# Pablete1234/parquet-floor

Measured on AMD Instinct MI355X. Metric: decoded GB/s + rows/s (node), lineitem-shape Snappy+dict, 1/2/4/8 GPUs, higher is better.
Workload: dtype u8; 1 GPU; lineitem SF1 x1 (6001215 rows x 1, 16 cols, 6 row groups of 1Mi rows), Snappy + dictionary, device-resident; row_groups_per_rank=6, compressed_page_bytes_rank0=217870360

## Files before the change

### parquet-floor_amd/csrc/pf_internal.h

```cpp
#pragma once
#include <stdint.h>

namespace pf {

struct PfOpts {
    int exec = 5;
    bool ba_fused = true;
    bool page_null = false;
    bool null_dict_lds = true;
    int null_stagger = 0;
    bool nest_timeout = false;
    uint32_t null_dcap = 0;
    bool piece_order = true;
    unsigned debug_skip = 0;
    int force_serial = 0;
    int force_redo = 0;
    bool exec_stream = false;
    bool zc = true;
    bool dl_kernel = true;
    bool h2d_kernel = false;
    int h2d_grid = 256;
    bool dl_stream = true;
    bool dl_prio = false;
    bool debug_plan = false;
    int64_t nest_seg = 0;
    bool nest_seg_set = false;
    bool dbp_par = true;
    int fix_shift = 1;
    int decode_grid = 32;
    int count_grid = 64;
};

enum : int32_t {
    PG_V2 = 1,
    PG_COMPRESSED = 2,
    PG_DICT = 4,
};

struct SnappyJob {
    const uint8_t* src;
// ... 116 lines not shown

constexpr uint32_t RT_CAP = 1024;
constexpr uint32_t RT_BYTES = 16 + 8 * RT_CAP;

constexpr uint32_t LT_BLOCK_RUNS = 512;
constexpr uint32_t LT_BT_WORDS = 8;
constexpr uint32_t NL_DST = 4096;
constexpr uint32_t NULL_DICT_LDS = 16384;
constexpr uint32_t NL_IST = 12288;
constexpr uint32_t NL_SLACK = 256;
struct NullCaps {
    uint32_t dcap, icap, dlds;
};
__host__ __device__ inline uint32_t lvl_table_cap(int32_t num_values) {
    return uint32_t(num_values) / 8u + 64u;
}

enum : int32_t { BA_OK = 0, BA_FALLBACK = 1, BA_SKIP = 2, BA_RELINK = 3 };
struct BaJob {
    const uint8_t* p;
    uint32_t* pos;
    uint32_t* len;
    int64_t* chars_out;
    uint32_t* cand;
    uint32_t* link1;
    uint32_t* link2;
    uint32_t* tile_cnt;
    int64_t count;
    uint32_t n;
    uint32_t n_cap;
    uint32_t n_tiles;
    int32_t chunk, page;
    int32_t state;
};

struct DevChunk {
    int32_t ptype, type_length, width, max_def, max_rep, repeated_def, list_null_def, codec;
    int32_t dict_page;
    int32_t first_page;
    int32_t n_pages;
    int32_t needs_count;
    int64_t num_entries;
    const uint8_t* dict_data;
    uint32_t* dict_pos;
    uint32_t* dict_len;
    int64_t dict_n;
    uint8_t* values;
    uint8_t* validity;
    int32_t* offsets;
    uint8_t* chars;
    int32_t* list_offsets;
    uint8_t* list_validity;
    uint8_t* def_levels;
    uint8_t* rep_levels;
    int64_t values_cap, chars_cap, slots_cap, rows_cap;
};

struct DevChunkResult {
    int64_t num_slots, num_values, num_rows, num_chars;
    int32_t status;
    int32_t err_page;
};

struct ScanChunk {
    const uint8_t* base;
    uint64_t size;
    int64_t num_values;
// ... 21 lines not shown
```

### parquet-floor_amd/csrc/pf_pages.hip

```cpp
#include <hip/hip_runtime.h>

#include "pf_device.h"
#include "pf_snappy_par.h"

namespace pf {

constexpr int NT = 256;

#ifdef PF_STAMPS
__device__ unsigned long long pf_pstamps[16];
#define PSTAMP(i, v) atomicAdd(&pf_pstamps[i], (unsigned long long)(v))
extern "C" int pf_debug_pstamps(unsigned long long* out, int n, int reset) {
    if (hipMemcpyFromSymbol(out, HIP_SYMBOL(pf_pstamps), sizeof(unsigned long long) * (n < 16 ? n : 16)) != hipSuccess) return -1;
    if (reset) {
        unsigned long long z[16] = {};
        if (hipMemcpyToSymbol(HIP_SYMBOL(pf_pstamps), z, sizeof z) != hipSuccess) return -1;
    }
    return 0;
}
#else
#define PSTAMP(i, v) ((void)0)
#endif
#ifndef PF_TILE
#define PF_TILE 512
// ... 529 lines not shown
            const uint32_t r = uint32_t(x - sb), ww = r >> 5;
            const uint32_t word = (C[ww] & L2[ww]) >> (r & 31u);
            const int64_t span = min(int64_t(32 - (r & 31u)), stop - x);
            if (word & (span >= 32 ? 0xffffffffu : ((1u << span) - 1u))) { bad = true; break; }
            x += span;
        }
        if (!bad && sv < wend && sv < int64_t(n)) {
            const uint32_t r = uint32_t(sv - sb);
            bad = !(((C[r >> 5] & L2[r >> 5]) >> (r & 31u)) & 1u);
        }
    }
    uint32_t tot;
    block_excl_scan<NT>(__popc(acc), tmp, tot);
    if (threadIdx.x == 0) J.tile_cnt[jt.y] = tot;
    if (__syncthreads_or(bad) && threadIdx.x == 0) atomicExch(&J.state, int32_t(BA_RELINK));
}

__global__ __launch_bounds__(NT) void k_ba_count(BaJob* __restrict__ jobs, const int2* __restrict__ tiles) {
    __shared__ uint32_t tmp[NT / 64];
    const int2 jt = tiles[blockIdx.x];
    const BaJob& J = jobs[jt.x];
    if (J.state != BA_OK) return;
    const uint32_t t0 = uint32_t(jt.y) * BA_TILE;
    if (t0 >= J.n) {
        if (threadIdx.x == 0) J.tile_cnt[jt.y] = 0;
        return;
    }
    const uint32_t wi = t0 / 32 + threadIdx.x;
    uint32_t tot;
    block_excl_scan<NT>(__popc(J.cand[wi] & J.link2[wi]), tmp, tot);
    if (threadIdx.x == 0) J.tile_cnt[jt.y] = tot;
}

__global__ __launch_bounds__(NT) void k_ba_scan(BaJob* __restrict__ jobs, int32_t fail_state) {
    __shared__ uint32_t tmp[NT / 64];
    BaJob& J = jobs[blockIdx.x];
    if (J.state != BA_OK) return;
    uint64_t run = 0;
    for (uint32_t b = 0; b < J.n_tiles; b += NT) {
        const uint32_t i = b + threadIdx.x;
        const uint32_t v = i < J.n_tiles ? J.tile_cnt[i] : 0u;
        uint32_t tot;
        const uint32_t ex = block_excl_scan<NT>(v, tmp, tot);
        if (i < J.n_tiles) J.tile_cnt[i] = uint32_t(run) + ex;
        run += tot;
    }
    if (threadIdx.x == 0 && int64_t(run) != J.count) {
        J.state = fail_state;
        PSTAMP(14, 1);
        PSTAMP(15, run > uint64_t(J.count) ? run - uint64_t(J.count) : 0);
    }
}

__global__ __launch_bounds__(NT) void k_ba_emit(BaJob* __restrict__ jobs, const int2* __restrict__ tiles) {
    __shared__ uint32_t tmp[NT / 64];
    const int2 jt = tiles[blockIdx.x];
    const BaJob& J = jobs[jt.x];
    if (J.state != BA_OK) return;
    const uint32_t n = J.n;
    const uint32_t t0 = uint32_t(jt.y) * BA_TILE;
    if (t0 >= n) return;
    const uint32_t wi = t0 / 32 + threadIdx.x;
    uint32_t m = J.cand[wi] & J.link2[wi];
    uint32_t tot;
    uint64_t k = uint64_t(J.tile_cnt[jt.y]) + block_excl_scan<NT>(__popc(m), tmp, tot);
    const uint64_t count = uint64_t(J.count);
    while (m) {
        const uint32_t q = wi * 32u + uint32_t(__ffs(m) - 1);
        m &= m - 1;
        if (k < count) {
            J.pos[k] = q + 4;
            if (J.len || k + 1 == count) {
                const uint32_t l = ld32le(J.p, q, n);
                if (J.len) J.len[k] = l;
                if (k + 1 == count && J.chars_out) *J.chars_out = int64_t(q) + 4 + int64_t(l) - 4 * int64_t(count);
            }
        }
        k++;
    }
}

__global__ __launch_bounds__(NT) void k_ba_verify(BaJob* __restrict__ jobs, const int2* __restrict__ tiles) {
    __shared__ uint32_t tmp[NT / 64];
    const int2 jt = tiles[blockIdx.x];
    BaJob& J = jobs[jt.x];
    if (J.state != BA_OK) return;
    const uint32_t n = J.n;
    const uint32_t t0 = uint32_t(jt.y) * BA_TILE;
    if (t0 >= n) return;
    const uint32_t wi = t0 / 32 + threadIdx.x;
    uint32_t m = J.cand[wi] & J.link2[wi];
// ... 93 lines not shown
    return 0;
}
#define BA_COUNT(i) (threadIdx.x == 0 ? (void)atomicAdd(&pf_ba_counts[i], 1ull) : (void)0)
#else
#define BA_COUNT(i) ((void)0)
#endif
__global__ __launch_bounds__(NT) void k_ba_fallback(BaJob* __restrict__ jobs, int n_jobs, DevChunkResult* res) {
    __shared__ BinWalkLds W;
    __shared__ long long s_chars;
    for (int j = blockIdx.x; j < n_jobs; j += gridDim.x) {
        BaJob& J = jobs[j];
        if (J.state == BA_RELINK) {
            if (threadIdx.x == 0) s_chars = 0;
            __syncthreads();
            const int64_t c = ba_relink_wg(J, W.scan);
            if (c > 0) atomicAdd(reinterpret_cast<unsigned long long*>(&s_chars), (unsigned long long)c);
            __syncthreads();
            if (c >= 0) {
                if (threadIdx.x == 0 && J.chars_out) *J.chars_out = s_chars;
                BA_COUNT(0);
                __syncthreads();
                continue;
            }
        } else if (J.state != BA_FALLBACK) {
            continue;
        }
        const int64_t t = binary_walk_wg(J.p, J.n, J.count, J.pos, J.len, W);
        BA_COUNT(1);
        if (threadIdx.x == 0) {
            if (t < 0) set_status(res, J.chunk, ST_CORRUPT, J.page);
            else if (J.chars_out) *J.chars_out = t;
        }
        __syncthreads();
    }
}

constexpr uint32_t DSTR_CAP = 256;
constexpr uint32_t FBLK = 4096;

__device__ __forceinline__ uint64_t* flat_block_chars(const DevPage& pg) {
    if (!pg.aux) return nullptr;
    const uintptr_t a = reinterpret_cast<uintptr_t>(pg.aux + pg.aux_cap + 1);
    return reinterpret_cast<uint64_t*>((a + 7) & ~uintptr_t(7));
}
__device__ __forceinline__ bool is_dict_enc(int e) { return e == 2 || e == 8; }

struct CountLds {
    LevelLds L;
    Piece pval[TILE];
    uint32_t ids[TILE];
    uint32_t scan_tmp[NT / 64];
    RleState sval;
    int npval, verr;
    unsigned long long chars_acc;
};

__device__ void count_page(const DevChunk* __restrict__ chunks, DevPage* pages, int pi, DevChunkResult* res, BaJob* bajobs,
                           CountLds& C) {
    LevelLds& L = C.L;
    Piece* pval = C.pval;
    uint32_t* ids = C.ids;
    uint32_t* scan_tmp = C.scan_tmp;
    RleState& sval = C.sval;
    int& npval = C.npval;
    int& verr = C.verr;
    unsigned long long& chars_acc = C.chars_acc;
// ... 1507 lines not shown
        }
        __syncthreads();
    }
    const bool direct = dval & (jf <= FB_WHOLE);
    const int err = flat_present_fixed(S, ck, pg, s, dict, boolean, enc, w, ids, ids_n, id_bw,
                                       uint64_t(pg.entry_start), e_begin, e_end, direct);
#ifdef PF_STAMPS
    if (tid == 0) { const unsigned long long dt_ = __builtin_amdgcn_s_memtime() - ft0; PSTAMP(1, dt_); PSTAMP(0, 1); atomicMax(&pf_pstamps[9], dt_); }
#endif
    if (tid == 0) {
        if (err) set_status(res, pg.chunk, ST_CORRUPT, pi);
        else if (ck.needs_count == 0)
            atomicAdd(reinterpret_cast<unsigned long long*>(&res[pg.chunk].num_values), (unsigned long long)(e_end - e_begin));
        atomicOr(&pg.done, DONE_FIXED);
    }
    return true;
}

__device__ __forceinline__ void null_fallback(int* fbq, int2 pbk) {
    if (threadIdx.x == 0) reinterpret_cast<int2*>(fbq + 4)[atomicAdd(fbq, 1)] = pbk;
}

#ifndef PF_FIXED_OCC
#define PF_FIXED_OCC 6
#endif
__global__ __launch_bounds__(NT, PF_FIXED_OCC) void k_flat_fixed(const DevChunk* __restrict__ chunks, DevPage* pages,
                                                              const int2* __restrict__ blocks, DevChunkResult* res, int* fbq) {
    __shared__ FixedLds S;
    const int2 pbk = blocks[blockIdx.x];
    if (!flat_fixed_block(S, chunks, pages, pbk, res)) null_fallback(fbq, pbk);
}

__device__ __forceinline__ void flat_block(FlatLds& S, const DevChunk* __restrict__ chunks, DevPage* pages, const int2 pbk,
                           DevChunkResult* res) {
    if (pbk.x < 0) return;
    const int pi = pbk.x;
    const uint32_t blk = uint32_t(pbk.y) & 0x0fffffffu;
    const uint32_t bsz = FBLK << (uint32_t(pbk.y) >> 28);
    DevPage& pg = pages[pi];
    const DevChunk& ck = chunks[pg.chunk];
    const int tid = threadIdx.x;
    if ((res[pg.chunk].status != 0) | (ck.max_rep != 0) | ((pg.done & (DONE_FIXED | DONE_NULL)) != 0)) return;
    Sections s;
    if (!page_sections(pg, ck, s)) return;
    const int enc = pg.encoding;
    const bool binary = ck.ptype == 6, boolean = ck.ptype == 0, dict = is_dict_enc(enc);
    const int w = ck.width;
    bool take = ck.max_def == 0 || s.def_rle;
    if (enc == 0) {
    } else if (dict) take = take && !boolean;
    else if (enc == 5) take = take && (ck.ptype == 1 || ck.ptype == 2) && pg.aux != nullptr;
    else take = false;
    if (!take) return;

    const int bwd = bit_width(ck.max_def);
    const uint32_t ne = uint32_t(pg.num_values);
    const int id_bw = (dict && s.val_n > 0) ? int(s.val[0]) : 0;
    const uint8_t* ids = dict && s.val_n > 0 ? s.val + 1 : s.val;
    const uint64_t ids_n = dict && s.val_n > 0 ? s.val_n - 1 : 0;
    const bool counted = ck.needs_count != 0;
    const uint64_t slot_base = uint64_t(pg.entry_start);
    if (blk > 0 && blk * bsz >= ne) return;
    const uint32_t* T = pg.runtab;
    uint32_t t0 = 0, t3 = 0;
    if (T != nullptr) { t0 = T[0]; t3 = T[3]; }
    const bool tab = (t3 == 1u) & (t0 <= uint32_t(RUN_CAP));
    if (tid == 0) S.allp = tab ? 1 : (ck.max_def == 0 ? 1 : all_present(s.def, s.def_n, bwd, ne, uint32_t(ck.max_def)));
    __syncthreads();
    const bool split = S.allp;
    if (!split && blk > 0) return;
    const uint32_t e_begin = split ? blk * bsz : 0u;
    const uint32_t e_end = split ? min(ne, e_begin + bsz) : ne;
#ifdef PF_STAMPS
    const unsigned long long ft0 = __builtin_amdgcn_s_memtime();
    if (tid == 0) { PSTAMP(0, 1); if (dict) PSTAMP(6, 1); if (binary) PSTAMP(7, 1); }
// ... 240 lines not shown
            else copy_chars_fast(S.coff, S.csrc, tv, tchars, sb, se, ck.chars + char_base, S.cv);
        }
        FSTAMP(15);
        if (ck.max_def > 0 && ck.validity) flush_bits(S.vbits, slot_base + e0, want, ck.validity);
        vidx += tv;
        char_base += tchars;
        __syncthreads();
#ifdef PF_STAMPS
        { const unsigned long long t_ = __builtin_amdgcn_s_memtime(); if (tid == 0) PSTAMP(5, t_ - ft1); ft1 = t_; }
#endif
    }
#ifdef PF_STAMPS
    if (tid == 0) {
        const unsigned long long dt_ = __builtin_amdgcn_s_memtime() - ft0;
        PSTAMP(1, dt_);
        atomicMax(&pf_pstamps[binary ? 8 : 9], dt_);
        if (!split) PSTAMP(10, 1);
    }
#endif
    if (tid == 0) {
        if (err) set_status(res, pg.chunk, ST_CORRUPT, pi);
        else if (!counted) atomicAdd(reinterpret_cast<unsigned long long*>(&res[pg.chunk].num_values),
                                     (unsigned long long)(vidx - e_begin));
        atomicOr(&pg.done, DONE_FLAT);
    }
}


#ifndef PF_FLAT_OCC
#define PF_FLAT_OCC 5
#endif
__global__ __launch_bounds__(NT, PF_FLAT_OCC) void k_flat_all(const DevChunk* __restrict__ chunks, DevPage* pages,
                                                 const int2* __restrict__ blocks, int n, const int* __restrict__ fbq,
                                                 DevChunkResult* res) {
    __shared__ union FlatAllLds {
        FixedLds f;
        FlatLds g;
    } S;
    if (int(blockIdx.x) >= n) {
        const int nq = fbq[0], g = int(gridDim.x) - n;
        for (int i = int(blockIdx.x) - n; i < nq; i += g) {
            const int2 pq = reinterpret_cast<const int2*>(fbq + 4)[i];
            if (!flat_fixed_block(S.f, chunks, pages, pq, res)) {
                __syncthreads();
                flat_block(S.g, chunks, pages, pq, res);
            }
            __syncthreads();
        }
        return;
    }
    const int2 pbk = blocks[blockIdx.x];
    if (flat_fixed_block(S.f, chunks, pages, pbk, res)) return;
    __syncthreads();
    flat_block(S.g, chunks, pages, pbk, res);
}

constexpr uint32_t LVL_STAGE = 4096;

__device__ __forceinline__ uint32_t lds_bits(const uint8_t* st, uint32_t bit, uint32_t k) {
    const uint32_t* w = reinterpret_cast<const uint32_t*>(st);
    const uint32_t wi = bit >> 5, sh = bit & 31u;
    const uint64_t v = uint64_t(w[wi]) | (uint64_t(w[wi + 1]) << 32);
    return uint32_t(v >> sh) & (k >= 32 ? 0xffffffffu : ((1u << k) - 1u));
}

__device__ __forceinline__ uint32_t lvl_run_at(const uint32_t* runs, uint32_t nr, uint32_t e) {
    uint32_t lo = 0, hi = nr;
    while (hi - lo > 1) {
        const uint32_t m = (lo + hi) >> 1;
        if (runs[4 * m] <= e) lo = m; else hi = m;
    }
    return lo;
}
__device__ inline uint32_t lvl_values_before(const uint32_t* runs, uint32_t r, uint32_t e, const uint8_t* stage,
                                             uint32_t woff, int bw, uint32_t maxd) {
    const uint32_t first = runs[4 * r], data = runs[4 * r + 1], cw = runs[4 * r + 2];
    const uint32_t before = e - first;
    uint32_t vb = runs[4 * r + 3];
    if (!(cw >> 31)) return vb + (data == maxd ? before : 0u);
    if (bw == 1) {
        for (uint32_t i = 0; i < before; i += 32) {
            const uint32_t k = min(32u, before - i), bb = woff * 8u + data + i;
            if (bb + k <= LVL_STAGE * 8u) vb += __popc(lds_bits(stage, bb, k));
        }
    } else {
        for (uint32_t i = 0; i < before; i++) {
            const uint32_t bb = woff * 8u + data + i * uint32_t(bw);
// ... 1305 lines not shown
    hipLaunchKernelGGL(k_count_seg, dim3(n_segs), dim3(NT), 0, st, d_chunks, d_pages, d_segs, d_res);
    hipLaunchKernelGGL(k_nest_scan, dim3(n), dim3(64), 0, st, d_chunks, d_pages, d_list, d_res);
    hipLaunchKernelGGL(k_nest_ids, dim3(n_segs), dim3(NT), 0, st, d_chunks, d_pages, d_segs, d_res);
    hipLaunchKernelGGL(k_nest_chars, dim3(n), dim3(64), 0, st, d_chunks, d_pages, d_list, d_res);
}
void launch_nest_decode(const DevChunk* d_chunks, DevPage* d_pages, const int2* d_segs, int n_segs, DevChunkResult* d_res,
                        hipStream_t st) {
    if (n_segs > 0) hipLaunchKernelGGL(k_decode_seg, dim3(n_segs), dim3(NT), 0, st, d_chunks, d_pages, d_segs, d_res);
}
void launch_count(const DevChunk* d_chunks, DevPage* d_pages, const int* d_list, int n, int n_flat, const int2* d_dblk, int n_dblk,
                  DevChunkResult* d_res, BaJob* d_bajobs, hipStream_t st, int idle_grid) {
    if (n <= 0) return;
    if (n_dblk > 0) hipLaunchKernelGGL(k_count_dict, dim3(n_dblk), dim3(NT), 0, st, d_chunks, d_pages, d_dblk, d_res);
    if (n_flat > 0) hipLaunchKernelGGL(k_count_flat, dim3(n_flat), dim3(NT), 0, st, d_chunks, d_pages, d_list, d_res, d_bajobs);
    hipLaunchKernelGGL(k_count, dim3(std::min(n, idle_grid)), dim3(NT), 0, st, d_chunks, d_pages, d_list, n, d_res, d_bajobs);
}
void launch_ba(BaJob* d_jobs, int n_jobs, const int2* d_tiles, int n_tiles, DevChunkResult* d_res, hipStream_t st,
               bool short_values) {
    if (n_jobs <= 0 || n_tiles <= 0) return;
    const bool fused = short_values;
    if (!fused) {
        hipLaunchKernelGGL(k_ba_cand, dim3(n_tiles), dim3(NT), 0, st, d_jobs, d_tiles);
        hipLaunchKernelGGL(k_ba_link, dim3(n_tiles), dim3(NT), 0, st, d_jobs, d_tiles, 1);
        hipLaunchKernelGGL(k_ba_link, dim3(n_tiles), dim3(NT), 0, st, d_jobs, d_tiles, 2);
        hipLaunchKernelGGL(k_ba_count, dim3(n_tiles), dim3(NT), 0, st, d_jobs, d_tiles);
    } else {
        hipLaunchKernelGGL(k_ba_tile, dim3(n_tiles), dim3(NT), 0, st, d_jobs, d_tiles);
    }
    hipLaunchKernelGGL(k_ba_scan, dim3(n_jobs), dim3(NT), 0, st, d_jobs, fused ? int32_t(BA_RELINK) : int32_t(BA_FALLBACK));
    hipLaunchKernelGGL(k_ba_emit, dim3(n_tiles), dim3(NT), 0, st, d_jobs, d_tiles);
    if (!fused) hipLaunchKernelGGL(k_ba_verify, dim3(n_tiles), dim3(NT), 0, st, d_jobs, d_tiles);
    hipLaunchKernelGGL(k_ba_fallback, dim3(std::min(n_jobs, 64)), dim3(NT), 0, st, d_jobs, n_jobs, d_res);
}
#ifdef PF_DIAG
__global__ __launch_bounds__(64) void k_debug_walk(const uint8_t* p, uint64_t n, int bw, uint32_t lo, uint32_t limit, int cap,
                                                    uint32_t pos0, uint32_t first0, uint32_t* out) {
    __shared__ Run R[RUN_CAP];
    __shared__ int s_nr;
    __shared__ uint32_t s_cov;
    __shared__ RunWalk s_st;
    const int tid = threadIdx.x;
    uint32_t* o1 = out;
    uint32_t* o2 = out + 5 + 4 * cap;
    if (tid == 0) {
        RunWalk st{pos0, first0};
        int nr = 0;
        uint32_t cov = 0;
        const int r = walk_runs(p, n, bw, lo, limit, R, cap, nr, cov, st);
        o1[0] = uint32_t(r); o1[1] = uint32_t(nr); o1[2] = cov; o1[3] = uint32_t(st.pos); o1[4] = st.first;
        for (int i = 0; i < nr; i++) { o1[5 + 4 * i] = R[i].first; o1[6 + 4 * i] = R[i].count; o1[7 + 4 * i] = R[i].data; o1[8 + 4 * i] = R[i].packed; }
        s_st = RunWalk{pos0, first0};
    }
    __syncthreads();
    const int r = wave_walk_runs(p, n, bw, lo, limit, R, cap, s_nr, s_cov, s_st, RunWalk{pos0, first0});
    __syncthreads();
    if (tid == 0) {
        o2[0] = uint32_t(r); o2[1] = uint32_t(s_nr); o2[2] = s_cov; o2[3] = uint32_t(s_st.pos); o2[4] = s_st.first;
    }
    for (int i = tid; i < s_nr; i += 64) { o2[5 + 4 * i] = R[i].first; o2[6 + 4 * i] = R[i].count; o2[7 + 4 * i] = R[i].data; o2[8 + 4 * i] = R[i].packed; }
}

extern "C" int pf_debug_walk_runs(const uint8_t* stream, uint64_t n, int bw, uint32_t lo, uint32_t limit, int cap,
                                  uint32_t pos0, uint32_t first0, uint32_t* out) {
    if (cap > int(RUN_CAP) || cap < 0) return -1;
    uint8_t* d = nullptr;
    uint32_t* o = nullptr;
// ... 53 lines not shown
                d[b] = g[tab[2 * k] + (b - tab[2 * k + 1])];
            }
        }
    }
}
void launch_snappy_litcopy(const SnappyJob* d_jobs, const int* d_list, int n, const int* d_fb, hipStream_t st) {
    if (n > 0) hipLaunchKernelGGL(k_snappy_litcopy, dim3(n, LC_SPLIT), dim3(NT), 0, st, d_jobs, d_list, d_fb);
}
void launch_snappy_head(SnappyJob* d_jobs, int n_jobs, DevPage* d_pages, const DevChunk* d_chunks, int* d_fb,
                        const DevChunkResult* d_res, hipStream_t st) {
    if (n_jobs > 0)
        hipLaunchKernelGGL(k_snappy_head, dim3((n_jobs + 63) / 64), dim3(64), 0, st, d_jobs, n_jobs, d_pages, d_chunks, d_fb,
                           d_res);
}
void launch_scan(DevChunk* d_chunks, DevPage* d_pages, const int* d_list, int n, DevChunkResult* d_res,
                 uint8_t* arena, uint64_t cap, unsigned long long* used, hipStream_t st) {
    if (n > 0) hipLaunchKernelGGL(k_scan, dim3(n), dim3(64), 0, st, d_chunks, d_pages, d_list, d_res, arena, cap, used);
}
void launch_runs(const DevChunk* d_chunks, DevPage* d_pages, const int* d_list, int n, DevChunkResult* d_res,
                 hipStream_t st) {
    if (n > 0) hipLaunchKernelGGL(k_runs, dim3(n), dim3(128), 0, st, d_chunks, d_pages, d_list, d_res);
}
void launch_lvl(const DevChunk* d_chunks, DevPage* d_pages, const int* d_list, int n, DevChunkResult* d_res,
                hipStream_t st, bool page_null, NullCaps nc) {
    if (n <= 0) return;
#ifdef PF_DIAG
    if (page_null) hipLaunchKernelGGL(k_page_null, dim3(n), dim3(PN_NT), 0, st, d_chunks, d_pages, d_list, d_res);
#else
    (void)page_null;
#endif
    hipLaunchKernelGGL(k_lvl, dim3(n), dim3(LT_NT), 0, st, d_chunks, d_pages, d_list, d_res, nc.dcap, nc.icap);
}
void launch_flat(const DevChunk* d_chunks, DevPage* d_pages, const int* d_list, int nfix, int n, int n4, int n8, int* d_fbq,
                 DevChunkResult* d_res, hipStream_t st, NullCaps nc, int stagger) {
    const int2* blocks = reinterpret_cast<const int2*>(d_list);
    const size_t dyn = size_t(nc.dcap) + 32u + nc.icap + 32u + nc.dlds;
    if (n4 > 0)
        hipLaunchKernelGGL(k_flat_null<4>, dim3(n4), dim3(NTN), dyn, st, d_chunks, d_pages, blocks + nfix + n, d_res, nc, stagger, d_fbq);
    if (n8 > 0)
        hipLaunchKernelGGL(k_flat_null<8>, dim3(n8), dim3(NTN), dyn, st, d_chunks, d_pages, blocks + nfix + n + n4, d_res, nc, stagger,
                           d_fbq);
    if (nfix > 0) hipLaunchKernelGGL(k_flat_fixed, dim3(nfix), dim3(NT), 0, st, d_chunks, d_pages, blocks, d_res, d_fbq);
    const int nq = nfix + n4 + n8;
    const int nqw = nq < 32 ? nq : 32;
    if (n + nqw > 0)
        hipLaunchKernelGGL(k_flat_all, dim3(n + nqw), dim3(NT), 0, st, d_chunks, d_pages, blocks + nfix, n, d_fbq, d_res);
}
void launch_decode(const DevChunk* d_chunks, DevPage* d_pages, const int* d_list, int n, int n_first,
                   DevChunkResult* d_res, hipStream_t st, int idle_grid) {
    const int g = std::min(n, std::max(idle_grid, n_first));
    if (n > 0) hipLaunchKernelGGL(k_decode, dim3(g), dim3(NT), 0, st, d_chunks, d_pages, d_list, n, d_res);
}

}
```

### parquet-floor_amd/csrc/pf_runtime.hip

```cpp
#include <hip/hip_runtime.h>

#include <algorithm>
#include <chrono>
#include <cstdio>
#include <cstdlib>
#include <cstring>
#include <memory>
#include <mutex>
#include <string>
#include <vector>

#include "pf_encode.h"
#include "pf_host.h"
#include "pf_snappy_par.h"
#include "pfloor.h"

namespace pf {
void launch_snappy(const SnappyJob*, int, const int2*, int, SnapWin*, SnapEnt*, uint32_t*, const int2*, int, uint32_t*,
                   int*, DevChunkResult*, int, int, hipStream_t);
void launch_snappy_parse(const SnappyJob*, int, const int2*, int, SnapWin*, SnapEnt*, uint32_t*, uint32_t*, int*, int,
                         hipStream_t);
void launch_snappy_exec(const SnappyJob*, int, const int2*, int, uint32_t*, int*, DevChunkResult*, int, hipStream_t);
void launch_ba(BaJob*, int, const int2*, int, DevChunkResult*, hipStream_t, bool);
void launch_snappy_head(SnappyJob*, int, DevPage*, const DevChunk*, int*, const DevChunkResult*, hipStream_t);
void launch_snappy_litcopy(const SnappyJob*, const int*, int, const int*, hipStream_t);
void launch_delta(const DevChunk*, DevPage*, const int*, int, int, DevChunkResult*, hipStream_t);
void launch_dlen(const DevChunk*, DevPage*, const int*, int, DevChunkResult*, hipStream_t);
void launch_dba_chars(const DevChunk*, DevPage*, const int*, int, DevChunkResult*, hipStream_t);
void launch_count(const DevChunk*, DevPage*, const int*, int, int, const int2*, int, DevChunkResult*, BaJob*, hipStream_t, int);
void launch_scan(DevChunk*, DevPage*, const int*, int, DevChunkResult*, uint8_t*, uint64_t, unsigned long long*, hipStream_t);
void launch_flat(const DevChunk*, DevPage*, const int*, int, int, int, int, int*, DevChunkResult*, hipStream_t, NullCaps, int);
void launch_lvl(const DevChunk*, DevPage*, const int*, int, DevChunkResult*, hipStream_t, bool, NullCaps);
void launch_runs(const DevChunk*, DevPage*, const int*, int, DevChunkResult*, hipStream_t);
void launch_decode(const DevChunk*, DevPage*, const int*, int, int, DevChunkResult*, hipStream_t, int);
void launch_nest_lvl(const DevChunk*, DevPage*, const int*, int, int, DevChunkResult*, hipStream_t, bool);
void launch_nest_count(const DevChunk*, DevPage*, const int*, int, const int2*, int, DevChunkResult*, hipStream_t);
void launch_nest_decode(const DevChunk*, DevPage*, const int2*, int, DevChunkResult*, hipStream_t);
void launch_page_scan(const ScanChunk*, int, pf_page_desc*, ScanCrc*, ScanResult*, hipStream_t);
void launch_page_crc(const ScanCrc*, const int*, int, ScanResult*, int32_t*, hipStream_t);
}

using namespace pf;

namespace {

thread_local std::string g_err;

int fail(pf_ctx* ctx, int code, const std::string& msg);

struct DevBuf {
    void* p = nullptr;
    size_t cap = 0;
    hipError_t ensure(size_t n) {
        if (n <= cap) return hipSuccess;
        if (p) { (void)hipFree(p); p = nullptr; cap = 0; }
        size_t want = std::max<size_t>(n + n / 4, 1 << 20);
        hipError_t e = hipMalloc(&p, want);
        if (e == hipSuccess) cap = want;
        return e;
    }
    void release() { if (p) (void)hipFree(p); p = nullptr; cap = 0; }
};

struct HostBuf {
// ... 90 lines not shown
    int device = 0;
    pf::PfOpts opts;
    std::shared_ptr<Streams> streams;
    hipStream_t stream = nullptr;
    hipStream_t exec_stream = nullptr;
    hipEvent_t ev_fork = nullptr, ev_join = nullptr;
    bool zc = true;
    hipEvent_t ev[N_EVENTS] = {};
    hipEvent_t ev_done = nullptr;
    hipEvent_t ev_copy = nullptr;
    hipEvent_t ev_dl = nullptr;
    bool timing = true;
    std::string err;
    DevBuf d_in, d_scratch, d_out, d_bits, d_chars, d_meta, d_tokmap;
    DevBuf d_scan_in, d_scan;
    DevBuf d_enc, d_enc_sec, d_enc_out;
    std::vector<uint8_t> h_enc;
    HostBuf h_meta, h_res;
    HostBuf h_enc_slots;
    int n_chunks = 0;
    bool pending = false;
    bool copies_pending = false;
    bool tables_from_decode = false;
    bool timing_valid = false;
    std::vector<DevChunk> chunks;
    std::vector<DevPage> pages;
    std::vector<SnappyJob> jobs;
    std::vector<int> l_dictbin, l_delta, l_count, l_scan, l_flat, l_decode, l_runs, l_dlen, l_dba, l_lvl, l_djobs, l_nest, l_nseg,
        l_cdict;
    std::vector<int2> wins, pieces;
    std::vector<BaJob> bajobs;
    std::vector<int2> ba_tiles;
    int n_ba_dict = 0, n_ba_dict_tiles = 0;
    bool ba_short_dict = true, ba_short_data = true;
    uint32_t null_dict_lds = 0;
    bool meta_by_kernel = false;
    uint32_t null_dcap = 16, null_icap = 16;
    int max_snap_win = 1;
    uint32_t n_splits = 0;
    SnapWin* d_win = nullptr;
    SnapEnt* d_ent = nullptr;
    const uint32_t* d_last_splits = nullptr;
    uint32_t* d_lane_out = nullptr;
    std::vector<int64_t> host_status;
    std::vector<pf_column_info> info;
    size_t bits_bytes = 0;
    int n_decode_first = 0;
    int n_count_flat = 0;
    int n_flat_fixed = 0, n_flat_all = 0, n_null4 = 0, n_null8 = 0;
    size_t off_npub = 0, npub_bytes = 0;
    int max_nwin = 0, max_dbp_nwin = 0;
    size_t out_bytes = 0;
    size_t off_chunks = 0, off_pages = 0, off_jobs = 0, off_lists = 0, off_res = 0, meta_bytes = 0;
    size_t off_pieces = 0, off_splits = 0, off_fallback = 0, off_wins = 0, off_bajobs = 0, off_batiles = 0, off_nfbq = 0;
    uint64_t chars_need = 0;
    const uint8_t* d_bytes = nullptr;
    int reruns = 0;
};

namespace {

int fail(pf_ctx* ctx, int code, const std::string& msg) {
    if (ctx) ctx->err = msg;
    g_err = msg;
    return code;
}
// ... 76 lines not shown
                           ctx->opts.exec, ctx->exec_stream);
        HIPCHK(ctx, hipEventRecord(ctx->ev_join, ctx->exec_stream));
        HIPCHK(ctx, hipStreamWaitEvent(st, ctx->ev_join, 0));
    } else {
        launch_snappy_exec(d_jobs, int(ctx->jobs.size()), d_pieces, int(ctx->pieces.size()), d_splits, d_fallback, d_res,
                           ctx->opts.exec, st);
    }
    EVREC(ctx, ctx->ev[3], st);
    BaJob* d_bajobs = reinterpret_cast<BaJob*>(meta + ctx->off_bajobs);
    const int2* d_batiles = reinterpret_cast<const int2*>(meta + ctx->off_batiles);
    const int n_ba = int(ctx->bajobs.size()), n_bt = int(ctx->ba_tiles.size());
    (void)d_dictbin;
    if (!(skip & 4u)) launch_ba(d_bajobs, ctx->n_ba_dict, d_batiles, ctx->n_ba_dict_tiles, d_res, st, ctx->ba_short_dict && ctx->opts.ba_fused);
    EVREC(ctx, ctx->ev[4], st);
    launch_delta(d_chunks, d_pages, d_delta, int(ctx->l_delta.size()), ctx->max_dbp_nwin, d_res, st);
    EVREC(ctx, ctx->ev[5], st);
    if (!(skip & 8u)) launch_runs(d_chunks, d_pages, d_runs, int(ctx->l_runs.size()), d_res, st);
    const NullCaps ncaps{ctx->opts.null_dcap ? ctx->opts.null_dcap : ctx->null_dcap, ctx->null_icap,
                         ctx->opts.null_dict_lds ? ctx->null_dict_lds : 0u};
    if (!(skip & 8u)) launch_lvl(d_chunks, d_pages, d_lvl, int(ctx->l_lvl.size()), d_res, st, ctx->opts.page_null, ncaps);
    launch_dlen(d_chunks, d_pages, d_dlen, int(ctx->l_dlen.size()), d_res, st);
    EVREC(ctx, ctx->ev[6], st);
    launch_nest_lvl(d_chunks, d_pages, d_nest, n_nest, ctx->max_nwin, d_res, st, ctx->opts.nest_timeout);
    if (!(skip & 16u)) launch_count(d_chunks, d_pages, d_count, int(ctx->l_count.size()), ctx->n_count_flat, d_cdict, int(ctx->l_cdict.size() / 2),
                                       d_res, d_bajobs, st, ctx->opts.count_grid);
    launch_nest_count(d_chunks, d_pages, d_nest, n_nest, d_nseg, n_nseg, d_res, st);
    if (!(skip & 4u))
        launch_ba(d_bajobs + ctx->n_ba_dict, n_ba - ctx->n_ba_dict, d_batiles + ctx->n_ba_dict_tiles, n_bt - ctx->n_ba_dict_tiles,
                  d_res, st, ctx->ba_short_data && ctx->opts.ba_fused);
    EVREC(ctx, ctx->ev[7], st);
    launch_scan(d_chunks, d_pages, d_scan, int(ctx->l_scan.size()), d_res, static_cast<uint8_t*>(ctx->d_chars.p),
                ctx->d_chars.cap, used, st);
    EVREC(ctx, ctx->ev[8], st);
    if (!(skip & 32u))
        launch_flat(d_chunks, d_pages, d_flat, ctx->n_flat_fixed, ctx->n_flat_all, ctx->n_null4, ctx->n_null8,
                    reinterpret_cast<int*>(meta + ctx->off_nfbq), d_res, st, ncaps, ctx->opts.null_stagger);
    EVREC(ctx, ctx->ev[9], st);
    if (!(skip & 64u)) launch_decode(d_chunks, d_pages, d_decode, int(ctx->l_decode.size()), ctx->n_decode_first, d_res, st,
                                       ctx->opts.decode_grid);
    launch_nest_decode(d_chunks, d_pages, d_nseg, n_nseg, d_res, st);
    launch_dba_chars(d_chunks, d_pages, d_dba, int(ctx->l_dba.size()), d_res, st);
    EVREC(ctx, ctx->ev[10], st);
    HIPCHK(ctx, hipGetLastError());
    const size_t res_pad = align_up(sizeof(DevChunkResult) * ctx->n_chunks, 256);
    if (ctx->zc && ctx->h_res.d) {
        copy_words(ctx->h_res.d, meta + ctx->off_res, sizeof(DevChunkResult) * ctx->n_chunks,
                   static_cast<uint8_t*>(ctx->h_res.d) + res_pad, d_chunks, sizeof(DevChunk) * ctx->n_chunks, st);
    } else {
        HIPCHK(ctx, hipMemcpyAsync(ctx->h_res.p, meta + ctx->off_res, sizeof(DevChunkResult) * ctx->n_chunks,
                                   hipMemcpyDeviceToHost, st));
        HIPCHK(ctx, hipMemcpyAsync(static_cast<uint8_t*>(ctx->h_res.p) + res_pad, d_chunks, sizeof(DevChunk) * ctx->n_chunks,
                                   hipMemcpyDeviceToHost, st));
    }
    HIPCHK(ctx, hipEventRecord(ctx->ev_done, st));
    return PF_OK;
}

int plan_snappy(pf_ctx* ctx) {
    ctx->wins.clear();
    ctx->pieces.clear();
    ctx->n_splits = 0;
    ctx->max_snap_win = 1;
    uint32_t n_win = 0;
    size_t tw = 0, tp = 0;
    for (SnappyJob& jb : ctx->jobs) {
        jb.n_win = std::max<uint32_t>(1u, uint32_t((uint64_t(jb.src_len) + SNAP_WIN - 1) / SNAP_WIN));
        ctx->max_snap_win = std::max(ctx->max_snap_win, int(std::min<uint32_t>(jb.n_win, 1u << 20)));
        jb.n_pieces = std::max<uint32_t>(1u, uint32_t((uint64_t(jb.dst_len) + SNAP_BLOCK - 1) / SNAP_BLOCK));
        tw += jb.n_win;
// ... 424 lines not shown
    out->encode_ms = enc_ms;
    out->snappy_in = 0;
    out->snappy_out = 0;
    if (col->codec == PF_CODEC_SNAPPY)
        for (size_t i = 0; i < sections.size(); i++) {
            out->snappy_in += int64_t(sections[i].second);
            out->snappy_out += int64_t(bodies[i].size());
        }
    return PF_OK;
}

extern "C" {

int pf_abi_version(void) { return PF_ABI_VERSION; }

const char* pf_last_error(pf_ctx* ctx) { return ctx ? ctx->err.c_str() : g_err.c_str(); }

int pf_device_count(int* count) {
    if (!count) return fail(nullptr, PF_ERR_INVALID_ARG, "null count");
    int n = 0;
    hipError_t e = hipGetDeviceCount(&n);
    if (e != hipSuccess) { *count = 0; return fail(nullptr, PF_ERR_HIP, hipGetErrorString(e)); }
    *count = n;
    return PF_OK;
}

namespace {
#ifdef PF_DIAG
void opts_from_env(pf::PfOpts& o) {
    auto on = [](const char* name, bool dflt) { const char* e = std::getenv(name); return e ? e[0] == '1' : dflt; };
    auto num = [](const char* name, int dflt) { const char* e = std::getenv(name); return e ? std::atoi(e) : dflt; };
    o.exec = num("PF_EXEC", o.exec);
    o.ba_fused = on("PF_BA_FUSED", o.ba_fused);
    o.page_null = on("PF_PAGE_NULL", o.page_null);
    o.null_dict_lds = on("PF_NULL_DICT_LDS", o.null_dict_lds);
    o.nest_timeout = on("PF_DEBUG_NEST_TIMEOUT", o.nest_timeout);
    o.null_dcap = uint32_t(std::max(0, num("PF_NULL_DCAP", 0))) & ~15u;
    o.null_stagger = num("PF_DEBUG_NULL_STAGGER", o.null_stagger);
    o.piece_order = on("PF_PIECE_ORDER", o.piece_order);
    if (const char* e = std::getenv("PF_DEBUG_SKIP")) {
        const char* names[] = {"parse", "exec", "ba", "levels", "count", "flat", "decode"};
        for (int i = 0; i < 7; i++)
            if (std::strstr(e, names[i])) o.debug_skip |= 1u << i;
    }
    o.force_serial = num("PF_DEBUG_FORCE_SERIAL", o.force_serial);
    o.force_redo = num("PF_DEBUG_FORCE_REDO", o.force_redo);
    o.exec_stream = on("PF_EXEC_STREAM", o.exec_stream);
    o.zc = on("PF_ZC", o.zc);
    o.dl_kernel = on("PF_DL_KERNEL", o.dl_kernel);
    o.dl_stream = on("PF_DL_STREAM", o.dl_stream);
    o.h2d_kernel = on("PF_H2D_KERNEL", o.h2d_kernel);
    o.h2d_grid = std::max(1, num("PF_H2D_GRID", o.h2d_grid));
    o.dl_prio = on("PF_DL_PRIO", o.dl_prio);
    o.debug_plan = on("PF_DEBUG_PLAN", o.debug_plan);
    if (const char* e = std::getenv("PF_NEST_SEG")) {
        o.nest_seg = std::atoll(e);
        o.nest_seg_set = true;
    }
    o.dbp_par = on("PF_DBP_PAR", o.dbp_par);
    o.decode_grid = std::max(1, num("PF_DECODE_GRID", o.decode_grid));
    o.count_grid = std::max(1, num("PF_COUNT_GRID", o.count_grid));
    const int fb = num("PF_FIX_BLK", 8192);
    o.fix_shift = fb >= 16384 ? 2 : (fb >= 8192 ? 1 : 0);
}
#endif

// ... 299 lines not shown
                            }
                        }
                    }
                }
                pplan.push_back(pp);
                ctx->pages.push_back(pg);
            }
        }
        if (hs != 0) {
            while (int(ctx->pages.size()) > ck.first_page) { ctx->pages.pop_back(); pplan.pop_back(); }
            while (!ctx->jobs.empty() && ctx->jobs.back().chunk == c) ctx->jobs.pop_back();
            if (!ctx->l_dictbin.empty() && ctx->l_dictbin.back() == c) ctx->l_dictbin.pop_back();
            ck.n_pages = 0; ck.dict_page = -1; entries = 0;
        }
        if (ck.dict_page >= 0) ck.first_page = ck.dict_page + 1;
        ck.num_entries = entries;
        OutPlan& op = oplan[c];
        op = OutPlan{~size_t(0), ~size_t(0), ~size_t(0), ~size_t(0), ~size_t(0), ~size_t(0), ~size_t(0)};
        if (hs == 0) {
            if (ck.width > 0) op.values = take(out, size_t(entries) * ck.width);
            if (cd.max_def > 0) op.validity = take(bits, align_up((entries + 7) / 8, 4), 256);
            if (cd.physical_type == PF_BYTE_ARRAY) op.offsets = take(out, 4 * size_t(entries + 1));
            if (cd.max_rep == 1) {
                op.list_offsets = take(out, 4 * size_t(entries + 1));
                op.list_validity = take(bits, align_up((entries + 7) / 8, 4), 256);
            }
            if (cd.max_rep > 0) { op.def = take(out, entries); op.rep = take(out, entries); }
        }
    }
    mark();
    ctx->bajobs.clear();
    ctx->ba_tiles.clear();
    ctx->ba_short_dict = ctx->ba_short_data = true;
    constexpr uint64_t BA_SHORT = 48;
    std::vector<size_t> ba_bm;
    for (int pass = 0; pass < 2; pass++) {
        for (size_t i = 0; i < ctx->pages.size(); i++) {
            DevPage& pg = ctx->pages[i];
            const DevChunk& ck = ctx->chunks[pg.chunk];
            if (ck.ptype != PF_BYTE_ARRAY || ctx->host_status[pg.chunk] != 0) continue;
            const bool is_dict = pg.flags & PG_DICT;
            if (pass == 0 ? !is_dict : (is_dict || pg.encoding != PF_ENC_PLAIN)) continue;
            BaJob J{};
            J.n_cap = pg.body_len;
            J.n_tiles = std::max<uint32_t>(1u, (pg.body_len + BA_TILE_BYTES - 1) / BA_TILE_BYTES);
            J.chunk = pg.chunk;
            J.page = int32_t(i);
            J.state = BA_SKIP;
            const size_t words = size_t(J.n_tiles) * (BA_TILE_BYTES / 32);
            ba_bm.push_back(take(scratch, 4 * (3 * words + J.n_tiles), 256));
            const int rel = int(ctx->bajobs.size()) - (pass == 0 ? 0 : ctx->n_ba_dict);
            for (uint32_t t = 0; t < J.n_tiles; t++) ctx->ba_tiles.push_back(int2{rel, int(t)});
            if (pass == 1) pg.ba_job = int32_t(ctx->bajobs.size());
            if (uint64_t(pg.body_len) > BA_SHORT * uint64_t(std::max<int64_t>(1, pg.num_values)))
                (pass == 0 ? ctx->ba_short_dict : ctx->ba_short_data) = false;
            ctx->bajobs.push_back(J);
        }
        if (pass == 0) { ctx->n_ba_dict = int(ctx->bajobs.size()); ctx->n_ba_dict_tiles = int(ctx->ba_tiles.size()); }
    }
    mark();
    size_t chars_cap = std::max<size_t>(size_t(2 * chars_hint) + (16u << 20), ctx->chars_need);
    if (ctx->copies_pending) {
        if (out > ctx->d_out.cap || bits > ctx->d_bits.cap || chars_cap > ctx->d_chars.cap)
            HIPCHK(ctx, hipEventSynchronize(ctx->ev_copy));
        else
            HIPCHK(ctx, hipStreamWaitEvent(st, ctx->ev_copy, 0));
// ... 66 lines not shown
            if (pp.dx_off != ~0ull) {
                pg.dx = reinterpret_cast<uint64_t*>(S + pp.dx_off);
                ctx->l_dlen.push_back(int(i));
                if (pg.encoding == PF_ENC_DELTA_BYTE_ARRAY) ctx->l_dba.push_back(int(i));
            }
            DevChunk& ck = ctx->chunks[pg.chunk];
            if (pp.is_dict) {
                ck.dict_data = pg.body;
                if (ck.ptype == PF_BYTE_ARRAY) {
                    ck.dict_pos = reinterpret_cast<uint32_t*>(S + pp.aux_off);
                    ck.dict_len = ck.dict_pos + (pg.num_values + 1);
                }
            }
        }
    }
    for (size_t b = 0; b < ctx->bajobs.size(); b++) {
        BaJob& J = ctx->bajobs[b];
        const size_t words = size_t(J.n_tiles) * (BA_TILE_BYTES / 32);
        J.cand = reinterpret_cast<uint32_t*>(S + ba_bm[b]);
        J.link1 = J.cand + words;
        J.link2 = J.link1 + words;
        J.tile_cnt = J.link2 + words;
        const DevPage& pg = ctx->pages[J.page];
        if (int(b) < ctx->n_ba_dict) {
            const DevChunk& ck = ctx->chunks[J.chunk];
            J.p = pg.body;
            J.n = pg.body_len;
            J.count = ck.dict_n;
            J.pos = ck.dict_pos;
            J.len = ck.dict_len;
            J.state = ck.dict_n > 0 ? BA_OK : BA_SKIP;
        } else {
            J.pos = pg.aux;
        }
    }
    for (int c = 0; c < n_chunks; c++) {
        DevChunk& ck = ctx->chunks[c];
        const OutPlan& op = oplan[c];
        auto at = [](uint8_t* base, size_t off) { return off == ~size_t(0) ? nullptr : base + off; };
        ck.values = at(O, op.values);
        ck.validity = at(B, op.validity);
        ck.offsets = reinterpret_cast<int32_t*>(at(O, op.offsets));
        ck.list_offsets = reinterpret_cast<int32_t*>(at(O, op.list_offsets));
        ck.list_validity = at(B, op.list_validity);
        ck.def_levels = at(O, op.def);
        ck.rep_levels = at(O, op.rep);
        if (ctx->host_status[c] == 0) {
            if (ck.needs_count) ctx->l_scan.push_back(c);
        }
    }
    constexpr uint32_t STICKY_DICT = 64u << 10;
    std::vector<int> spread[4];
    std::vector<std::vector<int>> sticky[4];
    for (auto& v : sticky) v.resize(static_cast<size_t>(n_chunks));
    std::vector<int> decode_first, count_rest;
    for (size_t i = 0; i < ctx->pages.size(); i++) {
        const DevPage& pg = ctx->pages[i];
        if (pg.flags & PG_DICT) continue;
        const DevChunk& ck = ctx->chunks[pg.chunk];
        if (pg.encoding == PF_ENC_DELTA_BINARY_PACKED && pg.aux && ck.ptype != PF_BYTE_ARRAY) ctx->l_delta.push_back(int(i));
        if (ck.needs_count) (ck.ptype == PF_BYTE_ARRAY && ck.max_rep == 0 ? ctx->l_count : count_rest).push_back(int(i));
        if (ck.ptype == PF_BYTE_ARRAY && ck.max_rep == 0 && pg.runtab != nullptr &&
            (pg.encoding == PF_ENC_PLAIN_DICTIONARY || pg.encoding == PF_ENC_RLE_DICTIONARY)) {
            const int nb = std::max(1, int((int64_t(pg.num_values) + FLAT_BLK - 1) / FLAT_BLK));
            for (int b = 0; b < nb; b++) { ctx->l_cdict.push_back(int(i)); ctx->l_cdict.push_back(b); }
        }
// ... 623 lines not shown
```

Measured before the change: 377.3 decoded GB/s.

## Add compact path for non-null PLAIN byte-array pages writing chars and offsets directly

For PLAIN BYTE_ARRAY data pages with no repetition, where the boundary scan finds exactly num_values entries (so no nulls), the page is marked for a compact path. A new per-tile kernel strips the 4-byte length prefixes in LDS, writes the chars contiguously, fills offsets and validity bits, and marks the page DONE_FLAT. The usual ba_emit position/length emission and the flat_block gather for those pages are skipped. This saves an intermediate pass and the extra traffic for string columns. In exchange it adds a kernel launch and relies on the candidate and link bitmaps being exact.

```diff
diff --git a/parquet-floor_amd/csrc/pf_internal.h b/parquet-floor_amd/csrc/pf_internal.h
--- a/parquet-floor_amd/csrc/pf_internal.h
+++ b/parquet-floor_amd/csrc/pf_internal.h
@@ -3,9 +3,13 @@
 
 namespace pf {
 
+#ifndef PF_BA_COMPACT
+#define PF_BA_COMPACT 1
+#endif
 struct PfOpts {
     int exec = 5;
     bool ba_fused = true;
+    bool ba_compact = PF_BA_COMPACT != 0;
     bool page_null = false;
     bool null_dict_lds = true;
     int null_stagger = 0;
@@ -188,7 +192,10 @@
     uint32_t n_tiles;
     int32_t chunk, page;
     int32_t state;
-};
+    int32_t num_values;
+    int32_t compact;
+};
+enum : int32_t { BAC_NO = 0, BAC_MAYBE = 1, BAC_TAKEN = 2 };
 
 struct DevChunk {
     int32_t ptype, type_length, width, max_def, max_rep, repeated_def, list_null_def, codec;
diff --git a/parquet-floor_amd/csrc/pf_pages.hip b/parquet-floor_amd/csrc/pf_pages.hip
--- a/parquet-floor_amd/csrc/pf_pages.hip
+++ b/parquet-floor_amd/csrc/pf_pages.hip
@@ -585,6 +585,20 @@
     if (threadIdx.x == 0) J.tile_cnt[jt.y] = tot;
 }
 
+#ifdef PF_DIAG
+__device__ unsigned long long pf_ba_taken;
+extern "C" int pf_debug_ba_compact_pages(unsigned long long* out, int reset) {
+    if (hipMemcpyFromSymbol(out, HIP_SYMBOL(pf_ba_taken), sizeof(unsigned long long)) != hipSuccess) return -1;
+    if (reset) {
+        const unsigned long long z = 0;
+        if (hipMemcpyToSymbol(HIP_SYMBOL(pf_ba_taken), &z, sizeof z) != hipSuccess) return -1;
+    }
+    return 0;
+}
+#define BA_TAKEN_COUNT() ((void)atomicAdd(&pf_ba_taken, 1ull))
+#else
+#define BA_TAKEN_COUNT() ((void)0)
+#endif
 __global__ __launch_bounds__(NT) void k_ba_scan(BaJob* __restrict__ jobs, int32_t fail_state) {
     __shared__ uint32_t tmp[NT / 64];
     BaJob& J = jobs[blockIdx.x];
@@ -598,18 +612,26 @@
         if (i < J.n_tiles) J.tile_cnt[i] = uint32_t(run) + ex;
         run += tot;
     }
-    if (threadIdx.x == 0 && int64_t(run) != J.count) {
+    if (threadIdx.x != 0) return;
+    if (int64_t(run) != J.count) {
         J.state = fail_state;
         PSTAMP(14, 1);
         PSTAMP(15, run > uint64_t(J.count) ? run - uint64_t(J.count) : 0);
-    }
+        if (J.compact == BAC_MAYBE) J.compact = BAC_NO;
+        return;
+    }
+    if (J.compact != BAC_MAYBE) return;
+    if (J.count != int64_t(J.num_values)) { J.compact = BAC_NO; return; }
+    J.compact = BAC_TAKEN;
+    BA_TAKEN_COUNT();
+    if (J.chars_out) *J.chars_out = int64_t(J.n) - 4 * J.count;
 }
 
 __global__ __launch_bounds__(NT) void k_ba_emit(BaJob* __restrict__ jobs, const int2* __restrict__ tiles) {
     __shared__ uint32_t tmp[NT / 64];
     const int2 jt = tiles[blockIdx.x];
     const BaJob& J = jobs[jt.x];
-    if (J.state != BA_OK) return;
+    if ((J.state != BA_OK) | (J.compact == BAC_TAKEN)) return;
     const uint32_t n = J.n;
     const uint32_t t0 = uint32_t(jt.y) * BA_TILE;
     if (t0 >= n) return;
@@ -769,6 +791,118 @@
             else if (J.chars_out) *J.chars_out = t;
         }
         __syncthreads();
+    }
+}
+
+constexpr uint32_t BAC_IMG = BA_TILE + 32;
+__global__ __launch_bounds__(NT) void k_ba_compact(const BaJob* __restrict__ jobs, const int2* __restrict__ tiles,
+                                                   const DevChunk* __restrict__ chunks, DevPage* pages,
+                                                   const DevChunkResult* __restrict__ res) {
+    __shared__ __attribute__((aligned(16))) uint8_t stg[BA_STAGE];
+    __shared__ __attribute__((aligned(16))) uint32_t img[BAC_IMG / 4];
+    __shared__ uint32_t acc_w[NT + 1];
+    __shared__ uint32_t tmp[NT / 64];
+    const int2 jt = tiles[blockIdx.x];
+    const BaJob& J = jobs[jt.x];
+    if (J.compact != BAC_TAKEN) return;
+    const DevChunk& ck = chunks[J.chunk];
+    if (res[J.chunk].status != 0 || ck.chars == nullptr || ck.offsets == nullptr) return;
+    const uint32_t n = J.n;
+    const uint32_t t0 = uint32_t(jt.y) * BA_TILE;
+    if (t0 >= n) return;
+    const uint32_t tid = threadIdx.x;
+    DevPage& pg = pages[J.page];
+    if (jt.y == 0 && tid == 0) atomicOr(&pg.done, DONE_FLAT);
+    const uint32_t woff = ba_stage(stg, J.p, n, t0);
+    for (uint32_t i = tid; i < BAC_IMG / 16; i += NT) reinterpret_cast<u32x4*>(img)[i] = u32x4{0u, 0u, 0u, 0u};
+    const uint32_t wi = t0 / 32 + tid;
+    const uint32_t q0 = t0 + tid * 32u;
+    const uint32_t live = q0 >= n ? 0u : (n - q0 >= 32u ? 0xffffffffu : ((1u << (n - q0)) - 1u));
+    const uint32_t A = J.cand[wi] & J.link2[wi] & live;
+    acc_w[tid + 1] = A;
+    if (tid == 0) acc_w[0] = wi > 0 ? (J.cand[wi - 1] & J.link2[wi - 1]) : 0u;
+    __syncthreads();
+    const uint32_t prevA = acc_w[tid], lastA = acc_w[0];
+    const uint32_t P = (A | (A << 1) | (A << 2) | (A << 3) | (prevA >> 29) | (prevA >> 30) | (prevA >> 31)) | ~live;
+    const uint32_t nch = uint32_t(__popc(~P));
+    uint32_t tot;
+    const uint32_t ex = block_excl_scan<NT>(uint32_t(__popc(A)) | (nch << 16), tmp, tot);
+    const uint32_t r0 = J.tile_cnt[jt.y];
+    const uint32_t tile_acc = tot & 0xffffu, tile_ch = tot >> 16;
+    const uint32_t lead = (lastA >> 31) ? 3u : ((lastA >> 30) & 1u) ? 2u : ((lastA >> 29) & 1u) ? 1u : 0u;
+    const int64_t out0 = pg.char_start + int64_t(t0) + int64_t(lead) - 4 * int64_t(r0);
+    uint8_t* gout = ck.chars + out0;
+    const uint32_t sh = uint32_t(reinterpret_cast<uintptr_t>(gout) & 15u);
+    if (nch) {
+        const uint32_t a = woff + tid * 32u;
+        const uint32_t* d = reinterpret_cast<const uint32_t*>(stg + (a & ~3u));
+        const uint32_t s = a & 3u;
+        uint32_t D[9];
+        #pragma unroll
+        for (int i = 0; i < 9; i++) D[i] = d[i];
+        const uint32_t cloc = sh + (ex >> 16);
+        uint32_t wdx = cloc >> 2, fill = cloc & 3u;
+        uint64_t acc = 0;
+        #pragma unroll
+        for (int k = 0; k < 8; k++) {
+            const uint32_t e = __builtin_amdgcn_alignbyte(D[k + 1], D[k], s);
+            const uint32_t pm = (P >> (4 * k)) & 15u;
+            uint32_t v = e, cnt = 4;
+            if (pm) {
+                v = 0; cnt = 0;
+                #pragma unroll
+                for (int j = 0; j < 4; j++)
+                    if (!((pm >> j) & 1u)) { v |= ((e >> (8 * j)) & 0xffu) << (8 * cnt); cnt++; }
+            }
+            acc |= uint64_t(v) << (8 * fill);
+            fill += cnt;
+            if (fill >= 4) {
+                atomicOr(&img[wdx], uint32_t(acc));
+                acc >>= 32;
+                fill -= 4;
+                wdx++;
+            }
+        }
+        if (fill) atomicOr(&img[wdx], uint32_t(acc));
+    }
+    {
+        const int64_t count = J.count;
+        int64_t k = int64_t(r0) + int64_t(ex & 0xffffu);
+        int32_t* offs = ck.offsets + pg.entry_start;
+        for (uint32_t m = A; m;) {
+            const uint32_t q = q0 + uint32_t(__ffs(m) - 1);
+            m &= m - 1;
+            if (k >= 1 && k < count) offs[k] = int32_t(pg.char_start + int64_t(q) - 4 * k);
+            if (k + 1 == count) offs[count] = int32_t(pg.char_start + int64_t(n) - 4 * count);
+            k++;
+        }
+    }
+    if (ck.max_def > 0 && ck.validity && tile_acc) {
+        uint32_t* vb = reinterpret_cast<uint32_t*>(ck.validity);
+        const uint64_t b0 = uint64_t(pg.entry_start) + r0, b1 = b0 + tile_acc;
+        const uint64_t w0 = b0 >> 5, w1 = (b1 - 1) >> 5;
+        for (uint64_t w = w0 + tid; w <= w1; w += NT) {
+            uint32_t v = 0xffffffffu;
+            if (w == w0) v &= 0xffffffffu << (b0 & 31u);
+            if (w == w1) v &= 0xffffffffu >> (31u - uint32_t((b1 - 1) & 31u));
+            if (w == w0 || w == w1) atomicOr(vb + w, v);
+            else vb[w] = v;
+        }
+    }
+    __syncthreads();
+    {
+        uint8_t* gbase = gout - sh;
+        const uint32_t end = sh + tile_ch;
+        const uint32_t nchunk = (end + 15u) / 16u;
+        for (uint32_t c = tid; c < nchunk; c += NT) {
+            const uint32_t lo = 16u * c, hi = lo + 16u;
+            if (lo >= sh && hi <= end) {
+                *reinterpret_cast<u32x4*>(gbase + lo) = reinterpret_cast<const u32x4*>(img)[c];
+            } else {
+                const uint8_t* ib = reinterpret_cast<const uint8_t*>(img);
+                for (uint32_t b = max(lo, sh); b < min(hi, end); b++) gbase[b] = ib[b];
+            }
+        }
     }
 }
 
@@ -2342,7 +2476,7 @@
 }
 
 __device__ __forceinline__ void flat_block(FlatLds& S, const DevChunk* __restrict__ chunks, DevPage* pages, const int2 pbk,
-                           DevChunkResult* res) {
+                           DevChunkResult* res, const BaJob* __restrict__ bajobs) {
     if (pbk.x < 0) return;
     const int pi = pbk.x;
     const uint32_t blk = uint32_t(pbk.y) & 0x0fffffffu;
@@ -2351,6 +2485,7 @@
     const DevChunk& ck = chunks[pg.chunk];
     const int tid = threadIdx.x;
     if ((res[pg.chunk].status != 0) | (ck.max_rep != 0) | ((pg.done & (DONE_FIXED | DONE_NULL)) != 0)) return;
+    if (pg.ba_job >= 0 && bajobs[pg.ba_job].compact == BAC_TAKEN) return;
     Sections s;
     if (!page_sections(pg, ck, s)) return;
     const int enc = pg.encoding;
@@ -2657,7 +2792,7 @@
 #endif
 __global__ __launch_bounds__(NT, PF_FLAT_OCC) void k_flat_all(const DevChunk* __restrict__ chunks, DevPage* pages,
                                                  const int2* __restrict__ blocks, int n, const int* __restrict__ fbq,
-                                                 DevChunkResult* res) {
+                                                 DevChunkResult* res, const BaJob* __restrict__ bajobs) {
     __shared__ union FlatAllLds {
         FixedLds f;
         FlatLds g;
@@ -2668,7 +2803,7 @@
             const int2 pq = reinterpret_cast<const int2*>(fbq + 4)[i];
             if (!flat_fixed_block(S.f, chunks, pages, pq, res)) {
                 __syncthreads();
-                flat_block(S.g, chunks, pages, pq, res);
+                flat_block(S.g, chunks, pages, pq, res, bajobs);
             }
             __syncthreads();
         }
@@ -2677,7 +2812,7 @@
     const int2 pbk = blocks[blockIdx.x];
     if (flat_fixed_block(S.f, chunks, pages, pbk, res)) return;
     __syncthreads();
-    flat_block(S.g, chunks, pages, pbk, res);
+    flat_block(S.g, chunks, pages, pbk, res, bajobs);
 }
 
 constexpr uint32_t LVL_STAGE = 4096;
@@ -4049,6 +4184,10 @@
     if (!fused) hipLaunchKernelGGL(k_ba_verify, dim3(n_tiles), dim3(NT), 0, st, d_jobs, d_tiles);
     hipLaunchKernelGGL(k_ba_fallback, dim3(std::min(n_jobs, 64)), dim3(NT), 0, st, d_jobs, n_jobs, d_res);
 }
+void launch_ba_compact(const BaJob* d_jobs, const int2* d_tiles, int n_tiles, const DevChunk* d_chunks, DevPage* d_pages,
+                       const DevChunkResult* d_res, hipStream_t st) {
+    if (n_tiles > 0) hipLaunchKernelGGL(k_ba_compact, dim3(n_tiles), dim3(NT), 0, st, d_jobs, d_tiles, d_chunks, d_pages, d_res);
+}
 #ifdef PF_DIAG
 __global__ __launch_bounds__(64) void k_debug_walk(const uint8_t* p, uint64_t n, int bw, uint32_t lo, uint32_t limit, int cap,
                                                     uint32_t pos0, uint32_t first0, uint32_t* out) {
@@ -4168,7 +4307,7 @@
     hipLaunchKernelGGL(k_lvl, dim3(n), dim3(LT_NT), 0, st, d_chunks, d_pages, d_list, d_res, nc.dcap, nc.icap);
 }
 void launch_flat(const DevChunk* d_chunks, DevPage* d_pages, const int* d_list, int nfix, int n, int n4, int n8, int* d_fbq,
-                 DevChunkResult* d_res, hipStream_t st, NullCaps nc, int stagger) {
+                 DevChunkResult* d_res, hipStream_t st, NullCaps nc, int stagger, const BaJob* d_bajobs) {
     const int2* blocks = reinterpret_cast<const int2*>(d_list);
     const size_t dyn = size_t(nc.dcap) + 32u + nc.icap + 32u + nc.dlds;
     if (n4 > 0)
@@ -4180,7 +4319,7 @@
     const int nq = nfix + n4 + n8;
     const int nqw = nq < 32 ? nq : 32;
     if (n + nqw > 0)
-        hipLaunchKernelGGL(k_flat_all, dim3(n + nqw), dim3(NT), 0, st, d_chunks, d_pages, blocks + nfix, n, d_fbq, d_res);
+        hipLaunchKernelGGL(k_flat_all, dim3(n + nqw), dim3(NT), 0, st, d_chunks, d_pages, blocks + nfix, n, d_fbq, d_res, d_bajobs);
 }
 void launch_decode(const DevChunk* d_chunks, DevPage* d_pages, const int* d_list, int n, int n_first,
                    DevChunkResult* d_res, hipStream_t st, int idle_grid) {
diff --git a/parquet-floor_amd/csrc/pf_runtime.hip b/parquet-floor_amd/csrc/pf_runtime.hip
--- a/parquet-floor_amd/csrc/pf_runtime.hip
+++ b/parquet-floor_amd/csrc/pf_runtime.hip
@@ -22,6 +22,7 @@
                          hipStream_t);
 void launch_snappy_exec(const SnappyJob*, int, const int2*, int, uint32_t*, int*, DevChunkResult*, int, hipStream_t);
 void launch_ba(BaJob*, int, const int2*, int, DevChunkResult*, hipStream_t, bool);
+void launch_ba_compact(const BaJob*, const int2*, int, const DevChunk*, DevPage*, const DevChunkResult*, hipStream_t);
 void launch_snappy_head(SnappyJob*, int, DevPage*, const DevChunk*, int*, const DevChunkResult*, hipStream_t);
 void launch_snappy_litcopy(const SnappyJob*, const int*, int, const int*, hipStream_t);
 void launch_delta(const DevChunk*, DevPage*, const int*, int, int, DevChunkResult*, hipStream_t);
@@ -29,7 +30,7 @@
 void launch_dba_chars(const DevChunk*, DevPage*, const int*, int, DevChunkResult*, hipStream_t);
 void launch_count(const DevChunk*, DevPage*, const int*, int, int, const int2*, int, DevChunkResult*, BaJob*, hipStream_t, int);
 void launch_scan(DevChunk*, DevPage*, const int*, int, DevChunkResult*, uint8_t*, uint64_t, unsigned long long*, hipStream_t);
-void launch_flat(const DevChunk*, DevPage*, const int*, int, int, int, int, int*, DevChunkResult*, hipStream_t, NullCaps, int);
+void launch_flat(const DevChunk*, DevPage*, const int*, int, int, int, int, int*, DevChunkResult*, hipStream_t, NullCaps, int, const BaJob*);
 void launch_lvl(const DevChunk*, DevPage*, const int*, int, DevChunkResult*, hipStream_t, bool, NullCaps);
 void launch_runs(const DevChunk*, DevPage*, const int*, int, DevChunkResult*, hipStream_t);
 void launch_decode(const DevChunk*, DevPage*, const int*, int, int, DevChunkResult*, hipStream_t, int);
@@ -186,6 +187,7 @@
     std::vector<BaJob> bajobs;
     std::vector<int2> ba_tiles;
     int n_ba_dict = 0, n_ba_dict_tiles = 0;
+    bool ba_compact_batch = false;
     bool ba_short_dict = true, ba_short_data = true;
     uint32_t null_dict_lds = 0;
     bool meta_by_kernel = false;
@@ -328,9 +330,13 @@
     launch_scan(d_chunks, d_pages, d_scan, int(ctx->l_scan.size()), d_res, static_cast<uint8_t*>(ctx->d_chars.p),
                 ctx->d_chars.cap, used, st);
     EVREC(ctx, ctx->ev[8], st);
-    if (!(skip & 32u))
+    if (!(skip & 32u)) {
+        if (ctx->ba_compact_batch && !(skip & 4u))
+            launch_ba_compact(d_bajobs + ctx->n_ba_dict, d_batiles + ctx->n_ba_dict_tiles, n_bt - ctx->n_ba_dict_tiles, d_chunks,
+                              d_pages, d_res, st);
         launch_flat(d_chunks, d_pages, d_flat, ctx->n_flat_fixed, ctx->n_flat_all, ctx->n_null4, ctx->n_null8,
-                    reinterpret_cast<int*>(meta + ctx->off_nfbq), d_res, st, ncaps, ctx->opts.null_stagger);
+                    reinterpret_cast<int*>(meta + ctx->off_nfbq), d_res, st, ncaps, ctx->opts.null_stagger, d_bajobs);
+    }
     EVREC(ctx, ctx->ev[9], st);
     if (!(skip & 64u)) launch_decode(d_chunks, d_pages, d_decode, int(ctx->l_decode.size()), ctx->n_decode_first, d_res, st,
                                        ctx->opts.decode_grid);
@@ -821,6 +827,7 @@
     auto num = [](const char* name, int dflt) { const char* e = std::getenv(name); return e ? std::atoi(e) : dflt; };
     o.exec = num("PF_EXEC", o.exec);
     o.ba_fused = on("PF_BA_FUSED", o.ba_fused);
+    o.ba_compact = on("PF_BA_COMPACT", o.ba_compact);
     o.page_null = on("PF_PAGE_NULL", o.page_null);
     o.null_dict_lds = on("PF_NULL_DICT_LDS", o.null_dict_lds);
     o.nest_timeout = on("PF_DEBUG_NEST_TIMEOUT", o.nest_timeout);
@@ -1186,6 +1193,7 @@
     ctx->bajobs.clear();
     ctx->ba_tiles.clear();
     ctx->ba_short_dict = ctx->ba_short_data = true;
+    ctx->ba_compact_batch = false;
     constexpr uint64_t BA_SHORT = 48;
     std::vector<size_t> ba_bm;
     for (int pass = 0; pass < 2; pass++) {
@@ -1318,6 +1326,10 @@
             J.state = ck.dict_n > 0 ? BA_OK : BA_SKIP;
         } else {
             J.pos = pg.aux;
+            J.num_values = pg.num_values;
+            const bool may = ctx->opts.ba_compact && ctx->opts.ba_fused && ctx->ba_short_data && ctx->chunks[J.chunk].max_rep == 0;
+            J.compact = may ? BAC_MAYBE : BAC_NO;
+            ctx->ba_compact_batch |= may;
         }
     }
     for (int c = 0; c < n_chunks; c++) {
```

Result: no change. 377.4 decoded GB/s, median of 2 (+0.0%).
